# adhammohamed1/Chandy-Lamport-Distributed-Snapshot-Algorithm

Measured on AMD Instinct MI355X. Metric: delivered packets/sec (whole node), higher is better.
Workload: dtype int32; 1 GPU; 8nodes-concurrent x 1,048,576: 8nodes.top + 8nodes-concurrent-snapshots.events, 2^20 instances split over the GPUs, Go delay streams; instances_total=1048576, instances_per_gpu=1048576, parallelism=instances sharded over 1 GPU(s), fifo_lds_slots=0

## Files before the change

### chandy-lamport-distributed-snapshot-algorithm_amd/csrc/cl_lanes.h

```cpp
#pragma once
#include "cl_engine.h"

namespace clsnap {
namespace lanes {

typedef __attribute__((address_space(3))) uint32_t lds_u32;
typedef const __attribute__((address_space(4))) ExecParams KPar;

__device__ __forceinline__ KPar* kpar() {
  auto* k = (const __attribute__((address_space(4))) char*)__builtin_amdgcn_kernarg_segment_ptr();
  asm volatile("" : "+s"(k));
  return (KPar*)k;
}

constexpr int rec_w(int D) { return D == 1 ? 2 : D <= 3 ? 4 : 8; }

struct Ctx {
  uint32_t lb;
  uint32_t lb2;
  uint32_t inst;
  uint32_t stride;
  uint32_t lrec;
  uint32_t plane8;
  int32_t draws;
  uint32_t dlast;
};

__device__ __forceinline__ lds_u32* lds_at(uint32_t byte) { return (lds_u32*)(size_t)byte; }
typedef __attribute__((address_space(3))) uint16_t lds_u16;
__device__ __forceinline__ lds_u16* lds16_at(uint32_t byte) { return (lds_u16*)(size_t)byte; }
struct Ctx;
__device__ __forceinline__ uint32_t fifo_rd(const Ctx& x, uint32_t i);
__device__ __forceinline__ void fifo_wr(const Ctx& x, uint32_t i, uint32_t v);
__device__ __forceinline__ uint32_t fifo_rd(const Ctx& x, uint32_t i) { return *lds16_at(x.lb2 + (i << 7)); }
__device__ __forceinline__ void fifo_wr(const Ctx& x, uint32_t i, uint32_t v) { *lds16_at(x.lb2 + (i << 7)) = (uint16_t)v; }
__device__ __forceinline__ uint32_t col_rd(const Ctx& x, uint32_t w) { return *lds_at(x.lb + (w << 8)); }
__device__ __forceinline__ void col_wr(const Ctx& x, uint32_t w, uint32_t v) { *lds_at(x.lb + (w << 8)) = v; }

template <class T>
struct Lds {
  static constexpr uint32_t CAP = 1u << T::CAPL;
  static constexpr uint32_t CAPM7 = (CAP - 1u) << 7;
  static constexpr uint32_t FW = ((uint32_t)T::E << T::CAPL) / 2;
  static constexpr uint32_t DUMMY = FW, DB = FW + 1;
};
__device__ __forceinline__ uint32_t due16(uint32_t e, int32_t time) {
  return (((((uint32_t)time - e) & 0xffu)) - 251u) >> 31;
}
__device__ __forceinline__ uint32_t e16_to_32(uint32_t e, int32_t time) {
  const uint32_t rt = (uint32_t)time + 5u - (((uint32_t)time + 5u - e) & 0xffu);
  return ((e & 0x8000u) << 16) | ((e >> 8) & 0x7fu) | (rt << 16);
}
__device__ __forceinline__ uint32_t e32_to_16(uint32_t e) {
  return ((e >> 16) & 0xffu) | ((e & 0x7fu) << 8) | ((e >> 16) & 0x8000u);
}

template <class T>
__device__ __forceinline__ uint32_t delays8(const Ctx& x, int32_t k) {
  const uint32_t w = min(Lds<T>::DB + ((uint32_t)k >> 3), x.dlast);
  const uint32_t lo = col_rd(x, w), hi = col_rd(x, w + 1);
  return __builtin_amdgcn_alignbit(hi, lo, ((uint32_t)k & 7u) * 4u);
}

template <class T>
__device__ __forceinline__ uint32_t node_off(const Ctx& x, uint32_t v) {
  (void)x;
  return v * (uint32_t)(rec_w(T::D) * 4 * (T::BLK ? 64 : 1));
}

__device__ __forceinline__ uint32_t plane_off(const Ctx& x, uint32_t sid) {
  return __umul24(sid, x.plane8) << 8;
}

template <class V>
__device__ __forceinline__ void st_at(V* base, uint32_t byte_off, V val) {
  *reinterpret_cast<V*>(reinterpret_cast<char*>(base) + byte_off) = val;
}

__device__ __forceinline__ void sched_fence() { __builtin_amdgcn_sched_barrier(0); }

template <class V>
__device__ __forceinline__ V opaque(V v) {
  asm volatile("" : "+v"(v));
  return v;
}

enum { TL_ROW, TL_PRO, TL_OPS, TL_LOOP, TL_WAIT, TL_EPI, TL_WAVES, TL_LOOPS, TL_NUM };
#if defined(CLSNAP_TIMELINE)
extern "C" {
__device__ unsigned long long clsnap_lanes_tl[2][64][TL_NUM];
}
struct Timeline {
  uint64_t last;
  uint32_t seg[TL_NUM];
  __device__ __forceinline__ static uint64_t now() {
    __builtin_amdgcn_sched_barrier(0);
    const uint64_t t = __builtin_amdgcn_s_memtime();
    __builtin_amdgcn_sched_barrier(0);
    return t;
  }
  __device__ __forceinline__ void begin() {
#pragma unroll
    for (int k = 0; k < TL_NUM; ++k) seg[k] = 0;
    seg[TL_WAVES] = 1;
    last = now();
  }
  __device__ __forceinline__ void mark(int k) {
    const uint64_t t = now();
    seg[k] += (uint32_t)(t - last);
    last = t;
  }
  __device__ __forceinline__ void count(int k) { seg[k] += 1; }
  __device__ __forceinline__ void drain() { __builtin_amdgcn_s_waitcnt(0x0f70); }
  __device__ __forceinline__ void flush(int kernel) {
    if (threadIdx.x == 0) {
#pragma unroll
      for (int k = 0; k < TL_NUM; ++k)
        atomicAdd(&clsnap_lanes_tl[kernel][blockIdx.x & 63u][k], (unsigned long long)seg[k]);
    }
  }
};
#else
struct Timeline {
  __device__ __forceinline__ void begin() {}
  __device__ __forceinline__ void mark(int) {}
  __device__ __forceinline__ void count(int) {}
  __device__ __forceinline__ void drain() {}
  __device__ __forceinline__ void flush(int) {}
};
#endif

template <int I>
struct IC {
  static constexpr int value = I;
};
template <int B, int E, class F>
__device__ __forceinline__ void sfor(F&& f) {
  if constexpr (B < E) {
    f(IC<B>{});
    sfor<B + 1, E>(f);
  }
}

template <class T>
struct State {
  int32_t tok[T::N];
  uint32_t hw[T::N][T::D];
  uint32_t cr[T::N][(T::D + 1) / 2];
  uint32_t pd[T::N][T::SW];
  uint32_t done[T::SW];
  int32_t time, draw, status, flag;
  uint32_t peek, push, ndone;
  bool alive;
};

template <class T>
__device__ __forceinline__ uint32_t cur_get(const State<T>& s, int v, int j) {
  return (s.cr[v][j >> 1] >> ((j & 1) * 16)) & 0xffffu;
}

template <class T>
__device__ __forceinline__ uint32_t pd_get(const State<T>& s, int v, uint32_t sid) {
  if constexpr (T::SW == 1) return s.pd[v][0];
  else return (sid & 8u) ? s.pd[v][1] : s.pd[v][0];
}
template <class T>
__device__ __forceinline__ void pd_set(State<T>& s, int v, uint32_t sid, uint32_t w) {
  if constexpr (T::SW == 1) {
    s.pd[v][0] = w;
  } else {
    const bool hi = (sid & 8u) != 0;
    s.pd[v][1] = hi ? w : s.pd[v][1];
    s.pd[v][0] = hi ? s.pd[v][0] : w;
  }
}

template <class T, bool SPILL>
__device__ __forceinline__ void push(const Ctx& x, uint32_t& hw, uint32_t ch, bool on, uint32_t pl16, int32_t kd,
                                     uint32_t delay, int32_t time, int32_t& nf) {
  using Ld = Lds<T>;
  const uint32_t cnt = hw & 0x7fu;
  const bool dly_ok = kd < x.draws;
  const bool live = on && dly_ok;
  bool ok = live && cnt < Ld::CAP;
  const uint32_t rt = (uint32_t)(time + 1 + (int32_t)delay);
  const uint32_t e = pl16 | (rt & 0xffu);
  const uint32_t slot = (x.lb2 | ((hw + (hw << 7)) & Ld::CAPM7)) + (ch << (T::CAPL + 7));
  *lds16_at(ok ? slot : x.lb + (Ld::DUMMY << 8)) = (uint16_t)e;
  if constexpr (SPILL) {
    if (__builtin_expect(live && cnt >= Ld::CAP, 0)) {
      KPar* p = kpar();
      const int32_t ocap = p->lay.ocap_log2;
      if (ocap >= 0 && cnt - Ld::CAP < (1u << ocap)) {
        const uint32_t om = (1u << ocap) - 1;
        uint32_t* hp = &p->ovh[ch * x.stride + x.inst];
        uint32_t h = 0;
        if (cnt == Ld::CAP) *hp = 0u;
        else h = *hp;
        p->ovf[((ch << ocap) + ((h + cnt - Ld::CAP) & om)) * x.stride + x.inst] =
            ((pl16 & 0x8000u) << 16) | ((pl16 >> 8) & 0x7fu) | (rt << 16);
        if (p->spill_flag) p->spill_flag[x.inst] = 1;
        ok = true;
      }
    }
  }
  if constexpr (!SPILL && T::PCAPL < T::CAPL) {
    if (__builtin_expect(ok && cnt >= (1u << T::PCAPL), 0)) {
      KPar* p = kpar();
      if (p->spill_flag) p->spill_flag[x.inst] = 1;
    }
  }
  hw += ok ? 1u : 0u;
  nf = (on && !ok) ? (dly_ok ? (int32_t)ST_FIFO_OVERFLOW : (int32_t)ST_DELAY_EXHAUSTED) : nf;
}

template <class T>
struct Guard {
  static constexpr uint32_t LIM = 1u << (T::PCAPL < T::CAPL ? T::PCAPL : T::CAPL);
  static constexpr uint32_t FULL = 0x7fu & ~(LIM - 1u);
};

template <class T>
__device__ __forceinline__ uint32_t sure_slot(const Ctx& x, uint32_t hw) {
  return x.lb2 | ((hw + (hw << 7)) & Lds<T>::CAPM7);
}
__device__ __forceinline__ uint32_t sure_entry(uint32_t pl16, uint32_t delay, int32_t time) {
  return pl16 | ((uint32_t)(time + 1 + (int32_t)delay) & 0xffu);
}

template <class T>
__device__ __forceinline__ void create_record(const Ctx& x, uint32_t* snod, const State<T>& s, int v, int arrive,
                                              uint32_t rb) {
  constexpr int RW = rec_w(T::D);
  uint32_t r[RW];
  r[0] = (uint32_t)s.tok[v];
#pragma unroll
  for (int j = 0; j < RW - 1; ++j) {
    const uint32_t c = (j < T::D && j < T::id(v)) ? cur_get(s, v, j < T::D ? j : 0) : 0u;
    r[1 + j] = j == arrive ? (c | (c << 16)) : c;
  }
  const uint32_t o = rb + node_off<T>(x, (uint32_t)v);
#if defined(CLSNAP_ABL_NOSTORE)
  if (o != 0xffffffffu) return;
#endif
  if constexpr (RW == 2) {
    st_at(reinterpret_cast<uint2*>(snod), o, make_uint2(r[0], r[1]));
  } else {
#pragma unroll
    for (int q = 0; q < RW; q += 4)
      st_at(reinterpret_cast<uint4*>(snod), o + 4u * q, make_uint4(r[q], r[q + 1], r[q + 2], r[q + 3]));
  }
}

template <class T>
__device__ __forceinline__ void resolve(State<T>& s) {
  if (s.flag != 0 && s.alive) {
    s.status = s.flag;
    s.alive = false;
  }
  s.flag = 0;
}

template <class T, bool SPILL>
__device__ __forceinline__ bool tick(const Ctx& x, State<T>& s, bool act) {
  constexpr int N = T::N, D = T::D;
  s.time += act ? 1 : 0;
  uint32_t e[N][D];
#pragma unroll
  for (int v = 0; v < N; ++v)
#pragma unroll
    for (int k = 0; k < D; ++k)
      if (k < T::od(v))
        e[v][k] = lds16_at(x.lb2 | (s.hw[v][k] & Lds<T>::CAPM7))[(T::off(v) + k) << (T::CAPL + 6)];
  uint32_t pk[N];
  uint32_t es[N];
#pragma unroll
  for (int v = 0; v < N; ++v) {
    pk[v] = 0;
    es[v] = 0;
    uint32_t sc = opaque(act ? 1u : 0u);
#pragma unroll
    for (int k = 0; k < D; ++k) {
      if (k >= T::od(v)) continue;
      const uint32_t w = s.hw[v][k];
      uint32_t ne;
      asm("v_min_u32 %0, %1, 1" : "=v"(ne) : "v"(w & 0x7fu));
      const uint32_t le = opaque(due16(e[v][k], s.time));
      const uint32_t lk = sc & ne;
      s.peek += lk;
      es[v] |= (sc - lk) << k;
      const uint32_t due = opaque(lk & le);
      if constexpr (SPILL) {
        if (__builtin_expect(due && (w & 0x7fu) > Lds<T>::CAP, 0)) {
          KPar* p = kpar();
          const uint32_t c = T::off(v) + k;
          const int32_t ocap = p->lay.ocap_log2;
          uint32_t* hp = &p->ovh[c * x.stride + x.inst];
          const uint32_t h = *hp;
          lds16_at(x.lb2 | (w & Lds<T>::CAPM7))[c << (T::CAPL + 6)] =
              (uint16_t)e32_to_16(p->ovf[((c << ocap) + h) * x.stride + x.inst]);
          *hp = (h + 1) & ((1u << ocap) - 1);
        }
      }
      s.hw[v][k] = w + __umul24(due, 0x7fu);
      const uint32_t val = e[v][k] | ((uint32_t)(k + 1) << 16);
      pk[v] = (val & (0u - due)) | (pk[v] & (due - 1u));
      sc -= due;
    }
    sched_fence();
  }
  {
    uint32_t any = 0;
#pragma unroll
    for (int v = 0; v < N; ++v) any |= pk[v];
    if (!__ballot(any != 0)) return true;
  }
  uint32_t tq[N];
  bool mkev = false;
  uint32_t* const snod = kpar()->snap_nod;
#pragma unroll
  for (int v = 0; v < N; ++v) {
    tq[v] = 0;
#pragma unroll
    for (int j = 0; j < D; ++j) {
      if (j >= T::id(v)) continue;
      const int sj = T::src(v, j);
      const uint32_t pkj = pk[sj];
      const bool m = (pkj >> 16) == (uint32_t)(T::oix(v, j) + 1);
      const bool mk = m && (pkj & 0x8000u);
      const bool tk = m && !(pkj & 0x8000u);
      s.tok[v] += tk ? (int32_t)((pkj >> 8) & 0x7fu) : 0;
      s.cr[v][j >> 1] += tk ? (1u << ((j & 1) * 16)) : 0u;
      mkev = mkev || mk;
      const uint32_t sid = (pkj >> 8) & 31u;
      const uint32_t sh = (sid & 7u) * 4u;
      uint32_t pw = pd_get(s, v, sid);
      const bool nz = ((pw >> sh) & 15u) != 0;
      const bool first = mk && !nz, later = mk && nz;
      pw += first ? ((uint32_t)T::id(v) << sh) : later ? (0u - (1u << sh)) : 0u;
      pd_set(s, v, sid, pw);
      if (T::od(v) > 0) {
        tq[v] |= first ? (0x80u | sid) << (8 * j) : 0u;
        if (T::src(v, j) < v) {
          s.peek += first ? (uint32_t)__builtin_popcount(es[v]) : 0u;
          es[v] = first ? 0u : es[v];
        }
      }
      const uint32_t rb = plane_off(x, sid) + x.lrec;
      if (first) create_record<T>(x, snod, s, v, j, rb);
#ifndef CLSNAP_ABL_NOSTORE
      if (later)
#else
      if (later && rb == 0xffffffffu)
#endif
        st_at(reinterpret_cast<uint16_t*>(snod), rb + node_off<T>(x, (uint32_t)v) + (uint32_t)(4 * (1 + j) + 2),
              (uint16_t)cur_get(s, v, j));
    }
    sched_fence();
  }
  if (__ballot(mkev)) {
#pragma unroll
    for (int w = 0; w < T::SW; ++w) {
      uint32_t all = 0x88888888u;
#pragma unroll
      for (int v = 0; v < N; ++v) {
        const uint32_t y = s.pd[v][w] ^ 0x11111111u;
        all &= ~(((y & 0x77777777u) + 0x77777777u) | y);
      }
      uint32_t fresh = all & 0x88888888u & ~s.done[w];
      if (fresh) {
        KPar* p = kpar();
        int32_t* tick_row = p->snap_tick + x.inst * (uint32_t)p->lay.s_cap;
        while (fresh) {
          const uint32_t b = (uint32_t)__builtin_ctz(fresh);
#ifndef CLSNAP_ABL_NOTICK
          tick_row[(uint32_t)w * 8u + (b >> 2)] = s.time;
#else
          if (s.time == -7) tick_row[(uint32_t)w * 8u + (b >> 2)] = s.time;
#endif
          s.ndone += 1;
          s.done[w] |= 1u << b;
          fresh &= fresh - 1u;
        }
      }
    }
  }
  bool trig = false;
#pragma unroll
  for (int v = 0; v < N; ++v) trig = trig || tq[v] != 0;
  if (__ballot(trig)) {
    uint32_t off[N];
    uint32_t acc = 0;
#pragma unroll
    for (int sv = 0; sv < N; ++sv) {
      off[sv] = acc;
#pragma unroll
      for (int k = 0; k < D; ++k) {
        if (k >= T::od(sv)) continue;
        const int r = T::dst(sv, k), q = T::ipos(sv, k);
        acc += ((tq[r] >> (8 * q + 7)) & 1u) * (uint32_t)T::od(r);
      }
    }
    uint32_t fv = 0xffu;
    int32_t fr = 0;
    auto one = [&](auto vc, auto fastc) {
      constexpr int v = decltype(vc)::value;
      constexpr bool FAST = decltype(fastc)::value != 0;
      if constexpr (T::od(v) > 0) {
        if (__ballot(tq[v] != 0)) {
          const uint32_t q = tq[v];
          const bool on = q != 0;
          const uint32_t lb = q ? (uint32_t)__builtin_ctz(q) & 24u : 0u;
          const uint32_t sid = (q >> lb) & 31u;
          tq[v] = q & ~(0xffu << lb);
          uint32_t oc[D];
#pragma unroll
          for (int j = 0; j < D; ++j) oc[j] = j < T::id(v) ? opaque(off[T::src(v, j < T::id(v) ? j : 0)]) : 0u;
          uint32_t o = oc[0];
#pragma unroll
          for (int j = 1; j < D; ++j)
            if (j < T::id(v)) o = lb == (uint32_t)(8 * j) ? oc[j] : o;
          const int32_t k0 = s.draw + (int32_t)o;
          const uint32_t dl = delays8<T>(x, k0);
          const uint32_t mpl = opaque(0x8000u | (sid << 8));
          bool hard = true;
          if constexpr (FAST) {
            uint32_t any = 0;
#pragma unroll
            for (int k = 0; k < D; ++k)
              if (k < T::od(v)) any |= s.hw[v][k];
            hard = on && (k0 + T::od(v) > x.draws || (any & Guard<T>::FULL) != 0);
          }
          if (!FAST || __builtin_expect(__ballot(hard) != 0, 0)) {
            int32_t nf = 0;
#pragma unroll
            for (int k = 0; k < D; ++k) {
              if (k >= T::od(v)) continue;
              push<T, SPILL>(x, s.hw[v][k], T::off(v) + k, on, mpl, k0 + k, (dl >> (4 * k)) & 15u, s.time, nf);
            }
            const bool take = nf != 0 && (uint32_t)v <= fv;
            fr = take ? nf : fr;
            fv = take ? (uint32_t)v : fv;
          } else {
            uint32_t sl[D], en[D];
#pragma unroll
            for (int k = 0; k < D; ++k) {
              if (k >= T::od(v)) continue;
              sl[k] = sure_slot<T>(x, s.hw[v][k]);
              en[k] = sure_entry(mpl, (dl >> (4 * k)) & 15u, s.time);
            }
            if (on) {
#pragma unroll
              for (int k = 0; k < D; ++k)
                if (k < T::od(v)) lds16_at(sl[k])[(T::off(v) + k) << (T::CAPL + 6)] = (uint16_t)en[k];
            }
            const uint32_t on01 = on ? 1u : 0u;
#pragma unroll
            for (int k = 0; k < D; ++k)
              if (k < T::od(v)) s.hw[v][k] += on01;
          }
        }
      }
    };
    sfor<0, N>([&](auto vc) { one(vc, IC<1>{}); });
    for (;;) {
      uint32_t rest = 0;
#pragma unroll
      for (int v = 0; v < N; ++v) rest |= tq[v];
      if (__builtin_expect(!__ballot(rest != 0), 1)) break;
      sfor<0, N>([&](auto vc) { one(vc, IC<0>{}); });
    }
    s.flag = s.flag ? s.flag : fr;
    s.draw += (int32_t)acc;
  }
  resolve(s);
  return false;
}

template <int N, class V>
__device__ __forceinline__ V pick_slot(const V (&a)[N], int32_t i) {
  V r = opaque(a[0]);
#pragma unroll
  for (int v = 1; v < N; ++v) r = v == i ? opaque(a[v]) : r;
  return r;
}
template <class T>
__device__ __forceinline__ uint32_t pick_hw(const State<T>& s, int32_t a, int32_t k) {
  uint32_t r = 0;
#pragma unroll
  for (int v = 0; v < T::N; ++v)
#pragma unroll
    for (int j = 0; j < T::D; ++j)
      if (j < T::od(v)) r = (v == a && j == k) ? opaque(s.hw[v][j]) : r;
  return r;
}

template <class T, bool SPILL>
__device__ __forceinline__ void send_one(const Ctx& x, State<T>& s, const Op& op) {
  const int32_t a = op.a, b = op.b;
  const int32_t tk = pick_slot<T::N>(s.tok, a);
  const bool insufficient = s.alive && tk < op.c;
  const bool go = s.alive && !insufficient && b >= 0;
  uint32_t hw = pick_hw(s, a, b);
  const uint32_t h0 = hw;
  int32_t nf = 0;
  const uint32_t ch = (uint32_t)(b >= 0 ? b : 0) + [&] {
    uint32_t o = 0;
#pragma unroll
    for (int v = 0; v < T::N; ++v) o = v == a ? T::off(v) : o;
    return o;
  }();
  push<T, SPILL>(x, hw, ch, go, (uint32_t)op.c << 8, s.draw, delays8<T>(x, s.draw) & 15u, s.time, nf);
  const uint32_t inc = hw - h0;
#pragma unroll
  for (int v = 0; v < T::N; ++v) {
    s.tok[v] -= (v == a && go) ? op.c : 0;
#pragma unroll
    for (int j = 0; j < T::D; ++j)
      if (j < T::od(v)) s.hw[v][j] += (v == a && j == b) ? inc : 0u;
  }
  s.flag = nf;
  if (s.alive) {
    if (insufficient) {
      s.status = ST_FATAL_INSUFFICIENT;
      s.alive = false;
    } else if (b < 0) {
      s.status = ST_FATAL_UNKNOWN_DEST;
      s.alive = false;
    } else {
      s.draw += 1;
    }
  }
  resolve(s);
}

template <class T, bool SPILL>
__device__ __forceinline__ void start_snapshot(const Ctx& x, State<T>& s, const Op& op) {
  constexpr int RW = rec_w(T::D);
  const int32_t a = op.a;
  const uint32_t sid = (uint32_t)op.b;
  const bool on = s.alive;
  int32_t id = 0, od = 0;
  uint32_t off = 0;
#pragma unroll
  for (int v = 0; v < T::N; ++v) {
    id = v == a ? T::id(v) : id;
    od = v == a ? T::od(v) : od;
    off = v == a ? T::off(v) : off;
  }
  const uint32_t nib = (id == 0 ? 15u : (uint32_t)id + 1u) << ((sid & 7u) * 4u);
#pragma unroll
  for (int v = 0; v < T::N; ++v)
#pragma unroll
    for (int w = 0; w < T::SW; ++w) s.pd[v][w] |= (on && v == a && (uint32_t)w == (sid >> 3)) ? nib : 0u;
  uint32_t r[RW];
  r[0] = (uint32_t)pick_slot<T::N>(s.tok, a);
#pragma unroll
  for (int j = 0; j < RW - 1; ++j) {
    uint32_t c = 0;
    if (j < T::D) {
#pragma unroll
      for (int v = 0; v < T::N; ++v)
        if (j < T::id(v)) c = v == a ? opaque(cur_get(s, v, j)) : c;
    }
    r[1 + j] = c;
  }
  if (on) {
    const uint32_t o = plane_off(x, sid) + x.lrec + node_off<T>(x, (uint32_t)a);
    uint32_t* snod = kpar()->snap_nod;
    if constexpr (RW == 2) {
      st_at(reinterpret_cast<uint2*>(snod), o, make_uint2(r[0], r[1]));
    } else {
#pragma unroll
      for (int q = 0; q < RW; q += 4)
        st_at(reinterpret_cast<uint4*>(snod), o + 4u * q, make_uint4(r[q], r[q + 1], r[q + 2], r[q + 3]));
    }
  }
  const uint32_t dl = delays8<T>(x, s.draw);
  int32_t nf = 0;
  uint32_t any = 0;
#pragma unroll
  for (int k = 0; k < T::D; ++k)
    if (k < od) any |= pick_hw(s, a, k);
  const bool hard = on && (s.draw + od > x.draws || (any & Guard<T>::FULL) != 0);
  if (__builtin_expect(__ballot(hard) != 0, 0)) {
#pragma unroll
    for (int k = 0; k < T::D; ++k) {
      if (k >= od) continue;
      uint32_t hw = pick_hw(s, a, k);
      const uint32_t h0 = hw;
      push<T, SPILL>(x, hw, off + (uint32_t)k, on, 0x8000u | (sid << 8), s.draw + k, (dl >> (4 * k)) & 15u, s.time,
                     nf);
      const uint32_t inc = hw - h0;
#pragma unroll
      for (int v = 0; v < T::N; ++v)
        if (k < T::od(v)) s.hw[v][k] += v == a ? inc : 0u;
    }
  } else {
    const uint32_t on01 = on ? 1u : 0u;
#pragma unroll
    for (int k = 0; k < T::D; ++k) {
      if (k >= od) continue;
      const uint32_t sl = sure_slot<T>(x, pick_hw(s, a, k)) + ((off + (uint32_t)k) << (T::CAPL + 7));
      const uint32_t en = sure_entry(0x8000u | (sid << 8), (dl >> (4 * k)) & 15u, s.time);
      if (on) *lds16_at(sl) = (uint16_t)en;
#pragma unroll
      for (int v = 0; v < T::N; ++v)
        if (k < T::od(v)) s.hw[v][k] += v == a ? on01 : 0u;
    }
  }
  s.flag = nf;
  if (s.alive) s.draw += op.c;
  resolve(s);
}

struct NoProg {
  static constexpr bool SPEC = false;
};

template <class T, bool SPILL, int A, int B, int C>
__device__ __forceinline__ void send_c(const Ctx& x, State<T>& s) {
  const bool insufficient = s.alive && s.tok[A] < C;
  const bool go = s.alive && !insufficient && B >= 0;
  int32_t nf = 0;
  if constexpr (B >= 0) {
    push<T, SPILL>(x, s.hw[A][B], T::off(A) + (uint32_t)B, go, (uint32_t)C << 8, s.draw, delays8<T>(x, s.draw) & 15u,
                   s.time, nf);
    s.tok[A] -= go ? C : 0;
  }
  s.flag = nf;
  if (s.alive) {
    if (insufficient) {
      s.status = ST_FATAL_INSUFFICIENT;
      s.alive = false;
    } else if (B < 0) {
      s.status = ST_FATAL_UNKNOWN_DEST;
      s.alive = false;
    } else {
      s.draw += 1;
    }
  }
  resolve(s);
}

template <class T, bool SPILL, int A, int SID, int C>
__device__ __forceinline__ void snap_c(const Ctx& x, State<T>& s) {
  constexpr int id = T::id(A), od = T::od(A);
  const bool on = s.alive;
  constexpr uint32_t nib = (id == 0 ? 15u : (uint32_t)id + 1u) << ((SID & 7) * 4);
  s.pd[A][SID >> 3] |= on ? nib : 0u;
  if (on) create_record<T>(x, kpar()->snap_nod, s, A, -1, plane_off(x, (uint32_t)SID) + x.lrec);
  int32_t nf = 0;
  if constexpr (od > 0) {
    const uint32_t dl = delays8<T>(x, s.draw);
    constexpr uint32_t mpl = 0x8000u | ((uint32_t)SID << 8);
    uint32_t any = 0;
#pragma unroll
    for (int k = 0; k < od; ++k) any |= s.hw[A][k];
    const bool hard = on && (s.draw + od > x.draws || (any & Guard<T>::FULL) != 0);
    if (__builtin_expect(__ballot(hard) != 0, 0)) {
#pragma unroll
      for (int k = 0; k < od; ++k)
        push<T, SPILL>(x, s.hw[A][k], T::off(A) + (uint32_t)k, on, mpl, s.draw + k, (dl >> (4 * k)) & 15u, s.time, nf);
    } else {
      uint32_t sl[od], en[od];
#pragma unroll
      for (int k = 0; k < od; ++k) {
        sl[k] = sure_slot<T>(x, s.hw[A][k]);
        en[k] = sure_entry(mpl, (dl >> (4 * k)) & 15u, s.time);
      }
      if (on) {
#pragma unroll
        for (int k = 0; k < od; ++k) lds16_at(sl[k])[(T::off(A) + k) << (T::CAPL + 6)] = (uint16_t)en[k];
      }
      const uint32_t on01 = on ? 1u : 0u;
#pragma unroll
      for (int k = 0; k < od; ++k) s.hw[A][k] += on01;
    }
  }
  s.flag = nf;
  if (s.alive) s.draw += C;
  resolve(s);
}

template <class T, bool SPILL>
__device__ __forceinline__ void tick_loop(const Ctx& x, State<T>& s, bool drain, int32_t a, int32_t b,
                                          int32_t n_started) {
  constexpr int N = T::N, D = T::D;
  constexpr int32_t kNoUntil = 0x7fffffff;
  int32_t until = drain ? kNoUntil : a;
  bool anyw = drain;
  for (int32_t iter = 0;; ++iter) {
    if (anyw) {
      const bool w = until == kNoUntil;
      if (w && (!s.alive || (int32_t)s.ndone >= n_started)) {
        until = iter + b;
      } else if (w && iter >= a) {
        s.status = ST_HANG;
        s.alive = false;
        until = iter;
      }
      anyw = __ballot(until == kNoUntil) != 0;
    }
    const bool act = s.alive && iter < until;
    if (!__ballot(act)) break;
    const bool idle = tick<T, SPILL>(x, s, act);
    if (idle && !anyw) {
      uint32_t q = 0;
#pragma unroll
      for (int v = 0; v < N; ++v)
#pragma unroll
        for (int k = 0; k < D; ++k)
          if (k < T::od(v)) q |= s.hw[v][k] & 0x7fu;
      if (!__ballot(q != 0)) {
        if (s.alive) s.time += max(0, until - (iter + 1));
        break;
      }
    }
  }
}

template <class T, bool SPILL, class P = NoProg>
__device__ __forceinline__ void program(const ExecParams& p, const Op* __restrict__ ops,
                                        const uint8_t* __restrict__ sched) {
  constexpr int N = T::N, D = T::D, RW = rec_w(T::D);
  const int32_t lane = threadIdx.x;
  const uint32_t slot = p.slot_base + blockIdx.x * (uint32_t)kWave + (uint32_t)lane;
  const bool valid = slot < (uint32_t)p.n_inst;
  const uint32_t inst = valid ? (p.inst_map ? (uint32_t)p.inst_map[slot] : slot) : 0u;
  const Layout& lay = p.lay;
  const uint32_t st = (uint32_t)p.stride;
  constexpr uint32_t capl = T::CAPL;
  const uint32_t nd = (uint32_t)(p.sched_row / 8);
  const Ctx x{(uint32_t)lane * 4u,
              ((uint32_t)lane & 31u) * 4u + ((uint32_t)lane >> 5) * 2u,
              inst,
              st,
              T::BLK ? 4u * (uint32_t)RW * ((slot >> 6) * 64u * (uint32_t)N + (slot & 63u))
                     : 4u * inst * (uint32_t)N * (uint32_t)RW,
              (4u * st * (uint32_t)N * (uint32_t)RW) >> 8,
              opaque((int32_t)(p.draws < 0x7fffffffLL ? p.draws : 0x7fffffffLL)),
              opaque(Lds<T>::DB + nd - 1)};

  Timeline tl;
  tl.begin();
  if (valid && p.sched_pk) {
    constexpr uint32_t kWordGroup = 16;
    const uint32_t* pk = p.sched_pk + ((size_t)(slot >> 6) * nd * 64u + (slot & 63u));
    for (uint32_t g = 0; g < nd; g += kWordGroup) {
      uint32_t b[kWordGroup];
#pragma unroll
      for (uint32_t j = 0; j < kWordGroup; ++j) b[j] = pk[(size_t)min(g + j, nd - 1) * 64u];
#pragma unroll
      for (uint32_t j = 0; j < kWordGroup; ++j) col_wr(x, Lds<T>::DB + min(g + j, nd - 1), b[j]);
    }
  } else if (valid) {
    const uint4* row = reinterpret_cast<const uint4*>(sched + (size_t)inst * p.sched_row);
    constexpr uint32_t kRowGroup = 8;
    const uint32_t nq = nd / 2;
    auto nib = [](uint32_t w) {
      return (w & 0xfu) | ((w >> 4) & 0xf0u) | ((w >> 8) & 0xf00u) | ((w >> 12) & 0xf000u);
    };
    for (uint32_t g = 0; g < nq; g += kRowGroup) {
      uint4 b[kRowGroup];
#pragma unroll
      for (uint32_t j = 0; j < kRowGroup; ++j) b[j] = row[min(g + j, nq - 1)];
#pragma unroll
      for (uint32_t j = 0; j < kRowGroup; ++j) {
        const uint32_t q = min(g + j, nq - 1);
        col_wr(x, Lds<T>::DB + 2 * q, nib(b[j].x) | (nib(b[j].y) << 16));
        col_wr(x, Lds<T>::DB + 2 * q + 1, nib(b[j].z) | (nib(b[j].w) << 16));
      }
    }
  }
  tl.mark(TL_ROW);

  State<T> s;
  s.flag = 0;
#pragma unroll
  for (int w = 0; w < T::SW; ++w) s.done[w] = 0;
#pragma unroll
  for (int v = 0; v < N; ++v) {
    s.tok[v] = p.lt.init_tok[v];
#pragma unroll
    for (int k = 0; k < D; ++k) s.hw[v][k] = 0;
#pragma unroll
    for (int k = 0; k < (D + 1) / 2; ++k) s.cr[v][k] = 0;
#pragma unroll
    for (int w = 0; w < T::SW; ++w) s.pd[v][w] = 0;
  }
  s.time = s.draw = s.status = 0;
  s.peek = s.push = s.ndone = 0;
  if (P::SPEC || p.fresh) {
    if (valid)
      for (int32_t sid = 0; sid < lay.s_cap; ++sid) p.snap_tick[inst * (uint32_t)lay.s_cap + sid] = -1;
  } else if (valid) {
    const uint32_t* S = p.state + inst;
    const uint32_t cap = 1u << capl;
#pragma unroll
    for (int v = 0; v < N; ++v) {
      const uint32_t b = (uint32_t)v * (uint32_t)(lay.priv + G_NUM);
      for (uint32_t q = 0; q < ((uint32_t)T::od(v) << capl); ++q)
        fifo_wr(x, (T::off(v) << capl) + q, e32_to_16(S[(b + lay.w_fifo + q) * st]));
#pragma unroll
      for (int k = 0; k < D; ++k) {
        const uint32_t lw = S[(b + lay.w_lnk + k) * st];
        if (k < T::od(v)) s.hw[v][k] = ((lw >> 8) & 0x7fu) | ((lw & 0xffu) << 7);
        if (k < T::id(v)) s.cr[v][k >> 1] |= (lw >> 16) << ((k & 1) * 16);
      }
      const uint32_t* R = S + (b + lay.priv) * st;
      s.tok[v] = (int32_t)R[G_TOKENS * st];
      const uint32_t started = R[G_STARTED * st];
      uint32_t pw[T::SW];
#pragma unroll
      for (int w = 0; w < T::SW; ++w) pw[w] = 0;
      for (int32_t sid = 0; sid < lay.s_cap; ++sid) {
        if (!((started >> sid) & 1u)) continue;
        const uint32_t pend = (S[(b + lay.w_pend + (sid >> 2)) * st] >> ((sid & 3) * 8)) & 0xffu;
        const uint32_t nib = (pend == 0 && T::id(v) == 0) ? 15u : pend + 1u;
#pragma unroll
        for (int w = 0; w < T::SW; ++w) pw[w] |= (w == (sid >> 3)) ? nib << ((sid & 7) * 4) : 0u;
      }
#pragma unroll
      for (int w = 0; w < T::SW; ++w) s.pd[v][w] = pw[w];
      if (v == 0) {
        s.time = (int32_t)R[G_TIME * st];
        s.draw = (int32_t)R[G_DRAW * st];
        s.status = (int32_t)R[G_STATUS * st];
      }
      s.peek += R[G_PEEK * st];
      s.push += R[G_PUSH * st];
    }
    const uint32_t* Dn = S + (uint32_t)N * (lay.priv + G_NUM) * st;
    for (int32_t sid = 0; sid < lay.s_cap; ++sid) {
      const uint32_t f = (int32_t)Dn[sid * st] >= N ? 8u << ((sid & 7) * 4) : 0u;
#pragma unroll
      for (int w = 0; w < T::SW; ++w) s.done[w] |= (w == (sid >> 3)) ? f : 0u;
    }
    s.ndone = Dn[lay.s_cap * st];
  }
  s.alive = valid && s.status == ST_OK;
  int32_t n_started = p.n_started_before;
  tl.mark(TL_PRO);

  if constexpr (P::SPEC) {
#pragma nounroll
    for (int32_t seg = 0; seg < P::NARM; ++seg) {
      bool drain = false;
      int32_t ta = 0, tb = 0;
      sfor<0, P::NARM>([&](auto gc) {
        constexpr int g = decltype(gc)::value;
        if (seg == g) {
          sfor<P::h0(g), P::h0(g + 1)>([&](auto hc) {
            constexpr int h = decltype(hc)::value;
            if constexpr (P::hk(h) == OP_SEND) send_c<T, SPILL, P::ha(h), P::hb(h), P::hc(h)>(x, s);
            else snap_c<T, SPILL, P::ha(h), P::hb(h), P::hc(h)>(x, s);
          });
          if constexpr (g < P::NSEG) {
            drain = P::td(g) != 0;
            ta = P::ta(g);
            tb = P::tb(g);
            n_started = P::ns(g);
          }
        }
      });
      if (P::NARM > P::NSEG && seg == P::NSEG) break;
      tl.mark(TL_OPS);
      tick_loop<T, SPILL>(x, s, drain, ta, tb, n_started);
      tl.mark(TL_LOOP);
      tl.drain();
      tl.mark(TL_WAIT);
      tl.count(TL_LOOPS);
    }
  }
  typedef const __attribute__((address_space(4))) Op COp;
  COp* cops = (COp*)ops;
  for (int32_t i = p.op_begin; !P::SPEC && i < p.op_end; ++i) {
    const Op op = cops[i];
    if (op.kind == OP_TICK || op.kind == OP_DRAIN) {
      tl.mark(TL_OPS);
      tick_loop<T, SPILL>(x, s, op.kind == OP_DRAIN, op.a, op.b, n_started);
      tl.mark(TL_LOOP);
      tl.drain();
      tl.mark(TL_WAIT);
      tl.count(TL_LOOPS);
      continue;
    }
    if (op.kind == OP_SEND) {
      send_one<T, SPILL>(x, s, op);
    } else if (op.kind == OP_SENDS) {
      for (int32_t q = 1; q <= op.a; ++q) send_one<T, SPILL>(x, s, (Op)cops[i + q]);
      i += op.a;
    } else if (op.kind == OP_SNAP) {
      start_snapshot<T, SPILL>(x, s, op);
      n_started++;
    }
  }
  tl.mark(TL_OPS);

  if (!valid) return;
  const uint32_t cap = 1u << capl;
  int32_t inflight = 0;
  uint32_t ptok = 0, pmk = 0, queued = 0;
#pragma unroll
  for (int v = 0; v < N; ++v) {
#pragma unroll
    for (int k = 0; k < D; ++k) {
      if (k < T::id(v)) ptok += cur_get(s, v, k);
      if (k >= T::od(v)) continue;
      const uint32_t w = s.hw[v][k], cnt = w & 0x7fu, head = (w >> 7) & 0xffu;
      const uint32_t c = T::off(v) + k;
      queued += cnt;
      for (uint32_t q = 0; q < cnt && q < cap; ++q) {
        const uint32_t e = fifo_rd(x, (c << capl) + ((head + q) & (cap - 1)));
        if (!(e & 0x8000u)) inflight += (int32_t)((e >> 8) & 0x7fu);
      }
      if (cnt > cap) {
        const uint32_t om = (1u << lay.ocap_log2) - 1;
        const uint32_t h = p.ovh[c * st + inst];
        for (uint32_t q = 0; q < cnt - cap; ++q) {
          const uint32_t e = p.ovf[((c << lay.ocap_log2) + ((h + q) & om)) * st + inst];
          if (!(e & kMarkerBit)) inflight += (int32_t)(e & 0xffffu);
        }
      }
    }
#pragma unroll
    for (int w = 0; w < T::SW; ++w)
      for (uint32_t m = s.pd[v][w]; m; m &= ~(15u << (__builtin_ctz(m) & ~3u))) {
        const uint32_t nib = (m >> (__builtin_ctz(m) & ~3u)) & 15u;
        pmk += (uint32_t)T::id(v) - (nib == 15u ? 0u : nib - 1u);
      }
  }
  int32_t* r = p.regs + (size_t)inst * R_NUM;
  r[R_TIME] = s.time;
  r[R_DRAW] = s.draw;
  r[R_STATUS] = s.status;
  r[R_NDONE] = (int32_t)s.ndone;
  r[R_PEEK] = (int32_t)s.peek;
  r[R_POP_TOK] = (int32_t)ptok;
  r[R_POP_MK] = (int32_t)pmk;
  const uint32_t pushes = ptok + pmk + queued;
  r[R_PUSH] = (int32_t)pushes;
  r[R_INFLIGHT_TOK] = inflight;
#pragma unroll
  for (int v = 0; v < N; ++v) p.fin_tok[inst * (uint32_t)N + v] = s.tok[v];
  tl.drain();
  tl.mark(TL_EPI);
  tl.flush(SPILL ? 1 : 0);
  if (P::SPEC || !p.save_state) return;
  uint32_t* S = p.state + inst;
#pragma unroll
  for (int v = 0; v < N; ++v) {
    const uint32_t b = (uint32_t)v * (uint32_t)(lay.priv + G_NUM);
    for (int32_t k = 0; k < lay.priv; ++k) S[(b + k) * st] = 0u;
    for (uint32_t q = 0; q < ((uint32_t)T::od(v) << capl); ++q)
      S[(b + lay.w_fifo + q) * st] = e16_to_32(fifo_rd(x, (T::off(v) << capl) + q), s.time);
#pragma unroll
    for (int k = 0; k < D; ++k) {
      uint32_t lw = k < T::id(v) ? cur_get(s, v, k) << 16 : 0u;
      if (k < T::od(v)) {
        const uint32_t w = s.hw[v][k];
        lw |= ((w >> 7) & (cap - 1)) | ((w & 0x7fu) << 8);
      }
      S[(b + lay.w_lnk + k) * st] = lw;
    }
    uint32_t started = 0;
    for (int32_t sid = 0; sid < lay.s_cap; ++sid) {
      uint32_t pw = 0;
#pragma unroll
      for (int w = 0; w < T::SW; ++w) pw = (w == (sid >> 3)) ? s.pd[v][w] : pw;
      const uint32_t nib = (pw >> ((sid & 7) * 4)) & 15u;
      if (!nib) continue;
      started |= 1u << sid;
      const uint32_t pend = nib == 15u ? 0u : nib - 1u;
      S[(b + lay.w_pend + (sid >> 2)) * st] |= pend << ((sid & 3) * 8);
    }
    uint32_t* R = S + (b + lay.priv) * st;
    R[G_TOKENS * st] = (uint32_t)s.tok[v];
    R[G_STARTED * st] = started;
    R[G_TIME * st] = (uint32_t)s.time;
    R[G_DRAW * st] = (uint32_t)s.draw;
    R[G_STATUS * st] = (uint32_t)s.status;
    R[G_PEEK * st] = v == 0 ? s.peek : 0u;
    R[G_POP_TOK * st] = v == 0 ? ptok : 0u;
    R[G_POP_MK * st] = v == 0 ? pmk : 0u;
    R[G_PUSH * st] = v == 0 ? pushes : 0u;
  }
  uint32_t* Dn = S + (uint32_t)N * (lay.priv + G_NUM) * st;
  for (int32_t sid = 0; sid < lay.s_cap; ++sid) {
    uint32_t c = 0;
#pragma unroll
    for (int v = 0; v < N; ++v) {
      uint32_t pw = 0;
#pragma unroll
      for (int w = 0; w < T::SW; ++w) pw = (w == (sid >> 3)) ? s.pd[v][w] : pw;
      c += ((pw >> ((sid & 7) * 4)) & 15u) == 1u ? 1u : 0u;
    }
    Dn[sid * st] = c;
  }
  Dn[lay.s_cap * st] = s.ndone;
}

}
}
```

Measured before the change: 82.22 billion packets/s.

## Pack per-channel FIFO head/count words for two nodes into packed 16-bit halves

Stores each pair of nodes' channel head/count state in one 32-bit register as two 16-bit halves, with a compile-time pairing table that groups nodes by out-degree. The per-tick FIFO peek and dequeue logic now runs on both halves at once with packed u16 vector ops (v_pk_min_u16, packed subtract, multiply and add), and the popcount of the skipped-edge mask is replaced by a direct count. The aim is to cut VGPR usage and VALU instruction count in the hot tick loop. In exchange the head counter is narrowed to 9 bits (CAPL<=9) and the push, snapshot and spill paths gain shift and extract overhead.

```diff
diff --git a/chandy-lamport-distributed-snapshot-algorithm_amd/csrc/cl_lanes.h b/chandy-lamport-distributed-snapshot-algorithm_amd/csrc/cl_lanes.h
--- a/chandy-lamport-distributed-snapshot-algorithm_amd/csrc/cl_lanes.h
+++ b/chandy-lamport-distributed-snapshot-algorithm_amd/csrc/cl_lanes.h
@@ -47,6 +47,18 @@
 __device__ __forceinline__ uint32_t due16(uint32_t e, int32_t time) {
   return (((((uint32_t)time - e) & 0xffu)) - 251u) >> 31;
 }
+typedef uint16_t us2 __attribute__((ext_vector_type(2)));
+__device__ __forceinline__ us2 as_us2(uint32_t v) { return __builtin_bit_cast(us2, v); }
+__device__ __forceinline__ uint32_t as_u32(us2 v) { return __builtin_bit_cast(uint32_t, v); }
+__device__ __forceinline__ uint32_t due16x2(uint32_t e2, us2 t2) {
+  const us2 d = as_us2(as_u32(t2 - as_us2(e2)) & 0x00ff00ffu) - (us2)(251);
+  return as_u32(d >> (us2)(15));
+}
+__device__ __forceinline__ uint32_t pk_min1(uint32_t c2) {
+  uint32_t r;
+  asm("v_pk_min_u16 %0, %1, 1 op_sel_hi:[1,0]" : "=v"(r) : "v"(c2));
+  return r;
+}
 __device__ __forceinline__ uint32_t e16_to_32(uint32_t e, int32_t time) {
   const uint32_t rt = (uint32_t)time + 5u - (((uint32_t)time + 5u - e) & 0xffu);
   return ((e & 0x8000u) << 16) | ((e >> 8) & 0x7fu) | (rt << 16);
@@ -143,9 +155,44 @@
 }
 
 template <class T>
+struct Pairs {
+  static constexpr int NP = (T::N + 1) / 2;
+  struct Tab {
+    int snd[NP][2];
+    int pr[T::N], hf[T::N];
+  };
+  static constexpr Tab make() {
+    Tab t{};
+    int ord[T::N] = {};
+    for (int v = 0; v < T::N; ++v) {
+      int i = v;
+      for (; i > 0 && T::od(ord[i - 1]) < T::od(v); --i) ord[i] = ord[i - 1];
+      ord[i] = v;
+    }
+    for (int p = 0; p < NP; ++p)
+      for (int h = 0; h < 2; ++h) {
+        const int v = 2 * p + h < T::N ? ord[2 * p + h] : -1;
+        t.snd[p][h] = v;
+        if (v >= 0) {
+          t.pr[v] = p;
+          t.hf[v] = h;
+        }
+      }
+    return t;
+  }
+  static constexpr Tab tab = make();
+  static constexpr int snd(int p, int h) { return tab.snd[p][h]; }
+  static constexpr int pr(int v) { return tab.pr[v]; }
+  static constexpr uint32_t sh(int v) { return 16u * (uint32_t)tab.hf[v]; }
+  static constexpr int od(int p, int h) { return tab.snd[p][h] < 0 ? 0 : T::od(tab.snd[p][h]); }
+  static constexpr int nk(int p) { return od(p, 0) > od(p, 1) ? od(p, 0) : od(p, 1); }
+  static constexpr uint32_t present(int p, int k) { return (k < od(p, 0) ? 1u : 0u) | (k < od(p, 1) ? 0x10000u : 0u); }
+};
+
+template <class T>
 struct State {
   int32_t tok[T::N];
-  uint32_t hw[T::N][T::D];
+  uint32_t hw[Pairs<T>::NP][T::D];
   uint32_t cr[T::N][(T::D + 1) / 2];
   uint32_t pd[T::N][T::SW];
   uint32_t done[T::SW];
@@ -155,6 +202,10 @@
 };
 
 template <class T>
+__device__ __forceinline__ uint32_t hw_get(const State<T>& s, int v, int k) {
+  return (s.hw[Pairs<T>::pr(v)][k] >> Pairs<T>::sh(v)) & 0xffffu;
+}
+template <class T>
 __device__ __forceinline__ uint32_t cur_get(const State<T>& s, int v, int j) {
   return (s.cr[v][j >> 1] >> ((j & 1) * 16)) & 0xffffu;
 }
@@ -176,16 +227,18 @@
 }
 
 template <class T, bool SPILL>
-__device__ __forceinline__ void push(const Ctx& x, uint32_t& hw, uint32_t ch, bool on, uint32_t pl16, int32_t kd,
-                                     uint32_t delay, int32_t time, int32_t& nf) {
+__device__ __forceinline__ void push(const Ctx& x, uint32_t& hw, uint32_t sh, uint32_t ch, bool on, uint32_t pl16,
+                                     int32_t kd, uint32_t delay, int32_t time, int32_t& nf) {
   using Ld = Lds<T>;
-  const uint32_t cnt = hw & 0x7fu;
+  static_assert(T::CAPL <= 9, "a ring's head slot must fit the half's 9-bit head counter");
+  const uint32_t h = hw >> sh;
+  const uint32_t cnt = h & 0x7fu;
   const bool dly_ok = kd < x.draws;
   const bool live = on && dly_ok;
   bool ok = live && cnt < Ld::CAP;
   const uint32_t rt = (uint32_t)(time + 1 + (int32_t)delay);
   const uint32_t e = pl16 | (rt & 0xffu);
-  const uint32_t slot = (x.lb2 | ((hw + (hw << 7)) & Ld::CAPM7)) + (ch << (T::CAPL + 7));
+  const uint32_t slot = (x.lb2 | ((h + (h << 7)) & Ld::CAPM7)) + (ch << (T::CAPL + 7));
   *lds16_at(ok ? slot : x.lb + (Ld::DUMMY << 8)) = (uint16_t)e;
   if constexpr (SPILL) {
     if (__builtin_expect(live && cnt >= Ld::CAP, 0)) {
@@ -210,7 +263,7 @@
       if (p->spill_flag) p->spill_flag[x.inst] = 1;
     }
   }
-  hw += ok ? 1u : 0u;
+  hw += ok ? 1u << sh : 0u;
   nf = (on && !ok) ? (dly_ok ? (int32_t)ST_FIFO_OVERFLOW : (int32_t)ST_DELAY_EXHAUSTED) : nf;
 }
 
@@ -221,8 +274,9 @@
 };
 
 template <class T>
-__device__ __forceinline__ uint32_t sure_slot(const Ctx& x, uint32_t hw) {
-  return x.lb2 | ((hw + (hw << 7)) & Lds<T>::CAPM7);
+__device__ __forceinline__ uint32_t sure_slot(const Ctx& x, uint32_t hw, uint32_t sh) {
+  const uint32_t h = hw >> sh;
+  return x.lb2 | ((h + (h << 7)) & Lds<T>::CAPM7);
 }
 __device__ __forceinline__ uint32_t sure_entry(uint32_t pl16, uint32_t delay, int32_t time) {
   return pl16 | ((uint32_t)(time + 1 + (int32_t)delay) & 0xffu);
@@ -265,56 +319,80 @@
 __device__ __forceinline__ bool tick(const Ctx& x, State<T>& s, bool act) {
   constexpr int N = T::N, D = T::D;
   s.time += act ? 1 : 0;
-  uint32_t e[N][D];
-#pragma unroll
-  for (int v = 0; v < N; ++v)
-#pragma unroll
-    for (int k = 0; k < D; ++k)
-      if (k < T::od(v))
-        e[v][k] = lds16_at(x.lb2 | (s.hw[v][k] & Lds<T>::CAPM7))[(T::off(v) + k) << (T::CAPL + 6)];
+  using Pr = Pairs<T>;
+  constexpr int NP = Pr::NP;
+  uint32_t e[NP][D];
+#pragma unroll
+  for (int p = 0; p < NP; ++p)
+#pragma unroll
+    for (int k = 0; k < D; ++k) {
+      if (k >= Pr::nk(p)) continue;
+      const uint32_t w = s.hw[p][k];
+      us2 ev = (us2)(0);
+      if (k < Pr::od(p, 0)) ev.x = lds16_at(x.lb2 | (w & Lds<T>::CAPM7))[(T::off(Pr::snd(p, 0)) + k) << (T::CAPL + 6)];
+      if (k < Pr::od(p, 1))
+        ev.y = lds16_at(x.lb2 | ((w >> 16) & Lds<T>::CAPM7))[(T::off(Pr::snd(p, 1)) + k) << (T::CAPL + 6)];
+      e[p][k] = as_u32(ev);
+    }
   uint32_t pk[N];
   uint32_t es[N];
-#pragma unroll
-  for (int v = 0; v < N; ++v) {
-    pk[v] = 0;
-    es[v] = 0;
-    uint32_t sc = opaque(act ? 1u : 0u);
+  uint32_t peek2 = 0;
+  uint32_t any = 0;
+  const us2 t2 = (us2)((uint16_t)s.time);
+  const uint32_t sc0 = opaque(act ? 0x10001u : 0u);
+#pragma unroll
+  for (int p = 0; p < NP; ++p) {
+    uint32_t pke = 0, pki = 0;
+    uint32_t lks = 0, scs = 0;
+    uint32_t sc = sc0;
 #pragma unroll
     for (int k = 0; k < D; ++k) {
-      if (k >= T::od(v)) continue;
-      const uint32_t w = s.hw[v][k];
-      uint32_t ne;
-      asm("v_min_u32 %0, %1, 1" : "=v"(ne) : "v"(w & 0x7fu));
-      const uint32_t le = opaque(due16(e[v][k], s.time));
+      if (k >= Pr::nk(p)) continue;
+      const uint32_t w = s.hw[p][k];
+      const uint32_t ne = pk_min1(w & 0x007f007fu);
+      const uint32_t le = opaque(due16x2(e[p][k], t2));
       const uint32_t lk = sc & ne;
-      s.peek += lk;
-      es[v] |= (sc - lk) << k;
+      lks += lk;
+      scs += Pr::present(p, k) == 0x10001u ? sc : sc & Pr::present(p, k);
       const uint32_t due = opaque(lk & le);
       if constexpr (SPILL) {
-        if (__builtin_expect(due && (w & 0x7fu) > Lds<T>::CAP, 0)) {
-          KPar* p = kpar();
-          const uint32_t c = T::off(v) + k;
-          const int32_t ocap = p->lay.ocap_log2;
-          uint32_t* hp = &p->ovh[c * x.stride + x.inst];
-          const uint32_t h = *hp;
-          lds16_at(x.lb2 | (w & Lds<T>::CAPM7))[c << (T::CAPL + 6)] =
-              (uint16_t)e32_to_16(p->ovf[((c << ocap) + h) * x.stride + x.inst]);
-          *hp = (h + 1) & ((1u << ocap) - 1);
+        if (__builtin_expect(due != 0 && (w & ((0x7fu & ~(Lds<T>::CAP - 1u)) * 0x10001u)) != 0, 0)) {
+#pragma unroll
+          for (int h = 0; h < 2; ++h) {
+            if (k >= Pr::od(p, h)) continue;
+            const uint32_t wh = w >> (16 * h);
+            if (((due >> (16 * h)) & 1u) && (wh & 0x7fu) > Lds<T>::CAP) {
+              KPar* kp = kpar();
+              const uint32_t c = T::off(Pr::snd(p, h)) + k;
+              const int32_t ocap = kp->lay.ocap_log2;
+              uint32_t* hp = &kp->ovh[c * x.stride + x.inst];
+              const uint32_t hd = *hp;
+              lds16_at(x.lb2 | (wh & Lds<T>::CAPM7))[c << (T::CAPL + 6)] =
+                  (uint16_t)e32_to_16(kp->ovf[((c << ocap) + hd) * x.stride + x.inst]);
+              *hp = (hd + 1) & ((1u << ocap) - 1);
+            }
+          }
         }
       }
-      s.hw[v][k] = w + __umul24(due, 0x7fu);
-      const uint32_t val = e[v][k] | ((uint32_t)(k + 1) << 16);
-      pk[v] = (val & (0u - due)) | (pk[v] & (due - 1u));
+      s.hw[p][k] = as_u32(as_us2(due) * (us2)(0x7f) + as_us2(w));
+      pke = as_u32(as_us2(e[p][k]) * as_us2(due) + as_us2(pke));
+      pki = as_u32(as_us2(due) * (us2)((uint16_t)(k + 1)) + as_us2(pki));
       sc -= due;
     }
+    peek2 += lks;
+    any |= pki;
+    const uint32_t es2 = scs - lks;
+#pragma unroll
+    for (int h = 0; h < 2; ++h) {
+      const int v = Pr::snd(p, h);
+      if (v < 0) continue;
+      pk[v] = __builtin_amdgcn_perm(pki, pke, h ? 0x07060302u : 0x05040100u);
+      es[v] = h ? es2 >> 16 : es2 & 0xffffu;
+    }
     sched_fence();
   }
-  {
-    uint32_t any = 0;
-#pragma unroll
-    for (int v = 0; v < N; ++v) any |= pk[v];
-    if (!__ballot(any != 0)) return true;
-  }
+  s.peek += (peek2 & 0xffffu) + (peek2 >> 16);
+  if (!__ballot(any != 0)) return true;
   uint32_t tq[N];
   bool mkev = false;
   uint32_t* const snod = kpar()->snap_nod;
@@ -342,7 +420,7 @@
       if (T::od(v) > 0) {
         tq[v] |= first ? (0x80u | sid) << (8 * j) : 0u;
         if (T::src(v, j) < v) {
-          s.peek += first ? (uint32_t)__builtin_popcount(es[v]) : 0u;
+          s.peek += first ? es[v] : 0u;
           es[v] = first ? 0u : es[v];
         }
       }
@@ -428,15 +506,16 @@
             uint32_t any = 0;
 #pragma unroll
             for (int k = 0; k < D; ++k)
-              if (k < T::od(v)) any |= s.hw[v][k];
-            hard = on && (k0 + T::od(v) > x.draws || (any & Guard<T>::FULL) != 0);
+              if (k < T::od(v)) any |= s.hw[Pr::pr(v)][k];
+            hard = on && (k0 + T::od(v) > x.draws || (any & (Guard<T>::FULL << Pr::sh(v))) != 0);
           }
           if (!FAST || __builtin_expect(__ballot(hard) != 0, 0)) {
             int32_t nf = 0;
 #pragma unroll
             for (int k = 0; k < D; ++k) {
               if (k >= T::od(v)) continue;
-              push<T, SPILL>(x, s.hw[v][k], T::off(v) + k, on, mpl, k0 + k, (dl >> (4 * k)) & 15u, s.time, nf);
+              push<T, SPILL>(x, s.hw[Pr::pr(v)][k], Pr::sh(v), T::off(v) + k, on, mpl, k0 + k, (dl >> (4 * k)) & 15u,
+                             s.time, nf);
             }
             const bool take = nf != 0 && (uint32_t)v <= fv;
             fr = take ? nf : fr;
@@ -446,7 +525,7 @@
 #pragma unroll
             for (int k = 0; k < D; ++k) {
               if (k >= T::od(v)) continue;
-              sl[k] = sure_slot<T>(x, s.hw[v][k]);
+              sl[k] = sure_slot<T>(x, s.hw[Pr::pr(v)][k], Pr::sh(v));
               en[k] = sure_entry(mpl, (dl >> (4 * k)) & 15u, s.time);
             }
             if (on) {
@@ -454,10 +533,10 @@
               for (int k = 0; k < D; ++k)
                 if (k < T::od(v)) lds16_at(sl[k])[(T::off(v) + k) << (T::CAPL + 6)] = (uint16_t)en[k];
             }
-            const uint32_t on01 = on ? 1u : 0u;
+            const uint32_t on01 = on ? 1u << Pr::sh(v) : 0u;
 #pragma unroll
             for (int k = 0; k < D; ++k)
-              if (k < T::od(v)) s.hw[v][k] += on01;
+              if (k < T::od(v)) s.hw[Pr::pr(v)][k] += on01;
           }
         }
       }
@@ -491,8 +570,16 @@
   for (int v = 0; v < T::N; ++v)
 #pragma unroll
     for (int j = 0; j < T::D; ++j)
-      if (j < T::od(v)) r = (v == a && j == k) ? opaque(s.hw[v][j]) : r;
+      if (j < T::od(v)) r = (v == a && j == k) ? opaque(hw_get(s, v, j)) : r;
   return r;
+}
+template <class T>
+__device__ __forceinline__ void bump_hw(State<T>& s, int32_t a, int32_t k, uint32_t inc) {
+#pragma unroll
+  for (int v = 0; v < T::N; ++v)
+#pragma unroll
+    for (int j = 0; j < T::D; ++j)
+      if (j < T::od(v)) s.hw[Pairs<T>::pr(v)][j] += (v == a && j == k) ? inc << Pairs<T>::sh(v) : 0u;
 }
 
 template <class T, bool SPILL>
@@ -510,15 +597,11 @@
     for (int v = 0; v < T::N; ++v) o = v == a ? T::off(v) : o;
     return o;
   }();
-  push<T, SPILL>(x, hw, ch, go, (uint32_t)op.c << 8, s.draw, delays8<T>(x, s.draw) & 15u, s.time, nf);
+  push<T, SPILL>(x, hw, 0u, ch, go, (uint32_t)op.c << 8, s.draw, delays8<T>(x, s.draw) & 15u, s.time, nf);
   const uint32_t inc = hw - h0;
 #pragma unroll
-  for (int v = 0; v < T::N; ++v) {
-    s.tok[v] -= (v == a && go) ? op.c : 0;
-#pragma unroll
-    for (int j = 0; j < T::D; ++j)
-      if (j < T::od(v)) s.hw[v][j] += (v == a && j == b) ? inc : 0u;
-  }
+  for (int v = 0; v < T::N; ++v) s.tok[v] -= (v == a && go) ? op.c : 0;
+  bump_hw(s, a, b, inc);
   s.flag = nf;
   if (s.alive) {
     if (insufficient) {
@@ -589,24 +672,19 @@
       if (k >= od) continue;
       uint32_t hw = pick_hw(s, a, k);
       const uint32_t h0 = hw;
-      push<T, SPILL>(x, hw, off + (uint32_t)k, on, 0x8000u | (sid << 8), s.draw + k, (dl >> (4 * k)) & 15u, s.time,
-                     nf);
-      const uint32_t inc = hw - h0;
-#pragma unroll
-      for (int v = 0; v < T::N; ++v)
-        if (k < T::od(v)) s.hw[v][k] += v == a ? inc : 0u;
+      push<T, SPILL>(x, hw, 0u, off + (uint32_t)k, on, 0x8000u | (sid << 8), s.draw + k, (dl >> (4 * k)) & 15u,
+                     s.time, nf);
+      bump_hw(s, a, k, hw - h0);
     }
   } else {
     const uint32_t on01 = on ? 1u : 0u;
 #pragma unroll
     for (int k = 0; k < T::D; ++k) {
       if (k >= od) continue;
-      const uint32_t sl = sure_slot<T>(x, pick_hw(s, a, k)) + ((off + (uint32_t)k) << (T::CAPL + 7));
+      const uint32_t sl = sure_slot<T>(x, pick_hw(s, a, k), 0u) + ((off + (uint32_t)k) << (T::CAPL + 7));
       const uint32_t en = sure_entry(0x8000u | (sid << 8), (dl >> (4 * k)) & 15u, s.time);
       if (on) *lds16_at(sl) = (uint16_t)en;
-#pragma unroll
-      for (int v = 0; v < T::N; ++v)
-        if (k < T::od(v)) s.hw[v][k] += v == a ? on01 : 0u;
+      bump_hw(s, a, k, on01);
     }
   }
   s.flag = nf;
@@ -624,8 +702,9 @@
   const bool go = s.alive && !insufficient && B >= 0;
   int32_t nf = 0;
   if constexpr (B >= 0) {
-    push<T, SPILL>(x, s.hw[A][B], T::off(A) + (uint32_t)B, go, (uint32_t)C << 8, s.draw, delays8<T>(x, s.draw) & 15u,
-                   s.time, nf);
+    push<T, SPILL>(x, s.hw[Pairs<T>::pr(A)][B], Pairs<T>::sh(A), T::off(A) + (uint32_t)B, go, (uint32_t)C << 8, s.draw,
+                   delays8<T>(x, s.draw) & 15u, s.time, nf);
+    s.hw[Pairs<T>::pr(A)][B] = opaque(s.hw[Pairs<T>::pr(A)][B]);
     s.tok[A] -= go ? C : 0;
   }
   s.flag = nf;
@@ -656,26 +735,27 @@
     constexpr uint32_t mpl = 0x8000u | ((uint32_t)SID << 8);
     uint32_t any = 0;
 #pragma unroll
-    for (int k = 0; k < od; ++k) any |= s.hw[A][k];
-    const bool hard = on && (s.draw + od > x.draws || (any & Guard<T>::FULL) != 0);
+    for (int k = 0; k < od; ++k) any |= s.hw[Pairs<T>::pr(A)][k];
+    const bool hard = on && (s.draw + od > x.draws || (any & (Guard<T>::FULL << Pairs<T>::sh(A))) != 0);
     if (__builtin_expect(__ballot(hard) != 0, 0)) {
 #pragma unroll
       for (int k = 0; k < od; ++k)
-        push<T, SPILL>(x, s.hw[A][k], T::off(A) + (uint32_t)k, on, mpl, s.draw + k, (dl >> (4 * k)) & 15u, s.time, nf);
+        push<T, SPILL>(x, s.hw[Pairs<T>::pr(A)][k], Pairs<T>::sh(A), T::off(A) + (uint32_t)k, on, mpl, s.draw + k,
+                       (dl >> (4 * k)) & 15u, s.time, nf);
     } else {
       uint32_t sl[od], en[od];
 #pragma unroll
       for (int k = 0; k < od; ++k) {
-        sl[k] = sure_slot<T>(x, s.hw[A][k]);
+        sl[k] = sure_slot<T>(x, s.hw[Pairs<T>::pr(A)][k], Pairs<T>::sh(A));
         en[k] = sure_entry(mpl, (dl >> (4 * k)) & 15u, s.time);
       }
       if (on) {
 #pragma unroll
         for (int k = 0; k < od; ++k) lds16_at(sl[k])[(T::off(A) + k) << (T::CAPL + 6)] = (uint16_t)en[k];
       }
-      const uint32_t on01 = on ? 1u : 0u;
-#pragma unroll
-      for (int k = 0; k < od; ++k) s.hw[A][k] += on01;
+      const uint32_t on01 = on ? 1u << Pairs<T>::sh(A) : 0u;
+#pragma unroll
+      for (int k = 0; k < od; ++k) s.hw[Pairs<T>::pr(A)][k] += on01;
     }
   }
   s.flag = nf;
@@ -708,10 +788,10 @@
     if (idle && !anyw) {
       uint32_t q = 0;
 #pragma unroll
-      for (int v = 0; v < N; ++v)
+      for (int p = 0; p < Pairs<T>::NP; ++p)
 #pragma unroll
         for (int k = 0; k < D; ++k)
-          if (k < T::od(v)) q |= s.hw[v][k] & 0x7fu;
+          if (k < Pairs<T>::nk(p)) q |= s.hw[p][k] & 0x007f007fu;
       if (!__ballot(q != 0)) {
         if (s.alive) s.time += max(0, until - (iter + 1));
         break;
@@ -783,12 +863,14 @@
   for (int v = 0; v < N; ++v) {
     s.tok[v] = p.lt.init_tok[v];
 #pragma unroll
-    for (int k = 0; k < D; ++k) s.hw[v][k] = 0;
-#pragma unroll
     for (int k = 0; k < (D + 1) / 2; ++k) s.cr[v][k] = 0;
 #pragma unroll
     for (int w = 0; w < T::SW; ++w) s.pd[v][w] = 0;
   }
+#pragma unroll
+  for (int q = 0; q < Pairs<T>::NP; ++q)
+#pragma unroll
+    for (int k = 0; k < D; ++k) s.hw[q][k] = 0;
   s.time = s.draw = s.status = 0;
   s.peek = s.push = s.ndone = 0;
   if (P::SPEC || p.fresh) {
@@ -805,7 +887,7 @@
 #pragma unroll
       for (int k = 0; k < D; ++k) {
         const uint32_t lw = S[(b + lay.w_lnk + k) * st];
-        if (k < T::od(v)) s.hw[v][k] = ((lw >> 8) & 0x7fu) | ((lw & 0xffu) << 7);
+        if (k < T::od(v)) s.hw[Pairs<T>::pr(v)][k] |= (((lw >> 8) & 0x7fu) | ((lw & 0xffu) << 7)) << Pairs<T>::sh(v);
         if (k < T::id(v)) s.cr[v][k >> 1] |= (lw >> 16) << ((k & 1) * 16);
       }
       const uint32_t* R = S + (b + lay.priv) * st;
@@ -908,7 +990,7 @@
     for (int k = 0; k < D; ++k) {
       if (k < T::id(v)) ptok += cur_get(s, v, k);
       if (k >= T::od(v)) continue;
-      const uint32_t w = s.hw[v][k], cnt = w & 0x7fu, head = (w >> 7) & 0xffu;
+      const uint32_t w = hw_get(s, v, k), cnt = w & 0x7fu, head = w >> 7;
       const uint32_t c = T::off(v) + k;
       queued += cnt;
       for (uint32_t q = 0; q < cnt && q < cap; ++q) {
@@ -959,7 +1041,7 @@
     for (int k = 0; k < D; ++k) {
       uint32_t lw = k < T::id(v) ? cur_get(s, v, k) << 16 : 0u;
       if (k < T::od(v)) {
-        const uint32_t w = s.hw[v][k];
+        const uint32_t w = hw_get(s, v, k);
         lw |= ((w >> 7) & (cap - 1)) | ((w & 0x7fu) << 8);
       }
       S[(b + lay.w_lnk + k) * st] = lw;
```

Result: faster. 86.49 billion packets/s (median of 6 runs) (+5.2%).
